# facebookarchive/Surround360

Measured on AMD Instinct MI355X. Metric: stereo-equirect frames/sec at 8K, 17-cam rig, higher is better.
Workload: dtype f32

## Files before the change

### surround360_amd/csrc/flow_kernels.hip

```cpp
#include "flow_kernels.hpp"

#include <stdexcept>

#include "devmath.hpp"

namespace s360 {

typedef float f4a8 __attribute__((ext_vector_type(4), aligned(8)));

__global__ __launch_bounds__(256) void k_resize_cubic_u8c4(const uchar4* __restrict__ src, int sw, int sh,
                                                           size_t sbs, uchar4* __restrict__ dst, int dw, int dh,
                                                           size_t dbs, double scx, double scy,
                                                           const uchar4* const* __restrict__ src_tab) {
  __shared__ int s_sx[32], s_sy[8];
  __shared__ short s_ax[32][4], s_ay[8][4];
  const int tid = threadIdx.y * blockDim.x + threadIdx.x;
  if (tid < 40) {
    const bool col = tid < 32;
    const int k = col ? tid : tid - 32;
    const int d = col ? min((int)(blockIdx.x * 32 + k), dw - 1) : min((int)(blockIdx.y * 8 + k), dh - 1);
    int s0;
    float f, cb[4];
    resize_coord(d, col ? scx : scy, &s0, &f);
    cubic_coeffs(f, cb);
    if (col) s_sx[k] = s0; else s_sy[k] = s0;
#pragma unroll
    for (int q = 0; q < 4; ++q) (col ? s_ax[k] : s_ay[k])[q] = (short)sat_s16(cv_round(cb[q] * 2048.f));
  }
  __syncthreads();
  const int dx = blockIdx.x * blockDim.x + threadIdx.x;
  const int dy = blockIdx.y * blockDim.y + threadIdx.y;
  if (dx >= dw || dy >= dh) return;
  src = src_tab ? src_tab[blockIdx.z] : src + sbs * blockIdx.z;
  dst += dbs * blockIdx.z;
  const int sx = s_sx[threadIdx.x], sy = s_sy[threadIdx.y];
  int ax[4], ay[4];
#pragma unroll
  for (int k = 0; k < 4; ++k) { ax[k] = s_ax[threadIdx.x][k]; ay[k] = s_ay[threadIdx.y][k]; }
  typedef short s16x2 __attribute__((ext_vector_type(2)));
  const s16x2 w01 = __builtin_bit_cast(s16x2, (unsigned)(ax[0] & 0xffff) | ((unsigned)ax[1] << 16));
  const s16x2 w23 = __builtin_bit_cast(s16x2, (unsigned)(ax[2] & 0xffff) | ((unsigned)ax[3] << 16));
  const int c0 = clip_idx(sx - 1, sw), c1 = clip_idx(sx, sw), c2 = clip_idx(sx + 1, sw), c3 = clip_idx(sx + 2, sw);
  int hx[4], hy[4], hz[4], hw[4];
#pragma unroll
  for (int r = 0; r < 4; ++r) {
    const unsigned* S = reinterpret_cast<const unsigned*>(src + (size_t)clip_idx(sy - 1 + r, sh) * sw);
    const unsigned p0 = S[c0], p1 = S[c1], p2 = S[c2], p3 = S[c3];
    int h[4];
#pragma unroll
    for (int ch = 0; ch < 4; ++ch) {
      const unsigned sel = 0x0c040c00u + ch * 0x00010001u;
      const s16x2 lo = __builtin_bit_cast(s16x2, __builtin_amdgcn_perm(p1, p0, sel));
      const s16x2 hi = __builtin_bit_cast(s16x2, __builtin_amdgcn_perm(p3, p2, sel));
      h[ch] = __builtin_amdgcn_sdot2(lo, w01, 0, false);
      h[ch] = __builtin_amdgcn_sdot2(hi, w23, h[ch], false);
    }
    hx[r] = h[0]; hy[r] = h[1]; hz[r] = h[2]; hw[r] = h[3];
  }
  uchar4 o;
  if (dx < (dw & ~1)) {
    const float scale = 1.f / (2048 * 2048);
    const float b0 = (float)ay[0] * scale, b1 = (float)ay[1] * scale, b2 = (float)ay[2] * scale, b3 = (float)ay[3] * scale;
    auto vf = [&](const int* hh) {
      float s = (float)hh[0] * b0;
      s = s + (float)hh[1] * b1;
      s = s + (float)hh[2] * b2;
      s = s + (float)hh[3] * b3;
      return (unsigned char)sat_u8(cv_round(s));
    };
    o.x = vf(hx); o.y = vf(hy); o.z = vf(hz); o.w = vf(hw);
  } else {
    auto vi = [&](const int* hh) {
      const int v = __mul24(hh[0], ay[0]) + __mul24(hh[1], ay[1]) + __mul24(hh[2], ay[2]) + __mul24(hh[3], ay[3]);
      return (unsigned char)sat_u8((v + (1 << 21)) >> 22);
    };
    o.x = vi(hx); o.y = vi(hy); o.z = vi(hz); o.w = vi(hw);
  }
  dst[(size_t)dy * dw + dx] = o;
}

__global__ __launch_bounds__(256) void k_gray_alpha(const uchar4* __restrict__ src, size_t n, size_t sbs,
                                                    float* __restrict__ gray, float* __restrict__ alpha,
                                                    size_t pbs) {
  const size_t i = (size_t)blockIdx.x * blockDim.x + threadIdx.x;
  if (i >= n) return;
  const uchar4 p = src[sbs * blockIdx.z + i];
  const float inv255 = (float)(1.0 / 255.0);
  const int g = (p.x * 1868 + p.y * 9617 + p.z * 4899 + (1 << 13)) >> 14;
  gray[pbs * blockIdx.z + i] = (float)g * inv255;
  alpha[pbs * blockIdx.z + i] = (float)p.w * inv255;
}

__global__ __launch_bounds__(256) void k_motion(const uchar4* __restrict__ cur, const uchar4* __restrict__ prev,
                                                size_t n, size_t sbs, float* __restrict__ motion, size_t pbs) {
  const size_t i = (size_t)blockIdx.x * blockDim.x + threadIdx.x;
  if (i >= n) return;
  const uchar4 a = cur[sbs * blockIdx.z + i], b = prev[sbs * blockIdx.z + i];
  const double s = fabs((double)((int)a.x - (int)b.x)) + fabs((double)((int)a.y - (int)b.y)) +
                   fabs((double)((int)a.z - (int)b.z));
  motion[pbs * blockIdx.z + i] = (float)(s / (double)(255.0f * 3.0f));
}

struct UpSrc {
  int sw, sh;
  size_t sbs;
  double scx, scy;
  float post_scale;
};
template <int R, int CN, int EPI, int SRC, int SB_TW = 64, int SB_TH = 16, int NT = 256>
__global__ __launch_bounds__(NT) void k_sepblur(const float* __restrict__ src, float* __restrict__ dst, int w, int h,
                                                 size_t bs , BlurTaps taps,
                                                 const float* __restrict__ A, FlowIdx idx,
                                                 const float2* __restrict__ Gp, void* __restrict__ recv,
                                                 float* const* __restrict__ dst_tab, UpSrc up,
                                                 unsigned* __restrict__ rowflags) {
  constexpr int IW = SB_TW + 2 * R, IH = SB_TH + 2 * R;
  constexpr int IWP = IW | 1;
  __shared__ __attribute__((aligned(8))) float s_in[IH][IWP][CN];
  __shared__ __attribute__((aligned(8))) float s_mid[IH][SB_TW + 1][CN];
  const int tid = threadIdx.y * blockDim.x + threadIdx.x;
  const TileId tile = xcd_tile();
  const int tx0 = tile.x * SB_TW, ty0 = tile.y * SB_TH;
  const int vecEnd = ((w * CN) / 8) * 8;
  constexpr int kColTasks = SB_TW * (SB_TH / 4);
  static_assert(EPI == 0 || kColTasks <= NT, "one column task per thread when the epilogue is prefetched");
  float pa0[4] = {0.f, 0.f, 0.f, 0.f}, pa1[4] = {0.f, 0.f, 0.f, 0.f}, pm[4] = {0.f, 0.f, 0.f, 0.f};
  float2 pg[4];
  if (EPI != 0 && tid < kColTasks) {
    const int lx = tid % SB_TW, ly0 = (tid / SB_TW) * 4, gx = tx0 + lx;
    const size_t b0 = bs * idx.i0[tile.z], b1 = bs * idx.i1[tile.z];
#pragma unroll
    for (int o = 0; o < 4; ++o) {
      const int gy = ty0 + ly0 + o;
      pg[o] = make_float2(0.f, 0.f);
      if (gx < w && gy < h) {
        const size_t off = (size_t)gy * w + gx;
        pa0[o] = A[b0 + off];
        pa1[o] = A[b1 + off];
        if (EPI == 3) pg[o] = Gp[b0 + off];
        if (EPI == 4) {
          pg[o] = Gp[bs * tile.z + off];
          pm[o] = static_cast<const float*>(recv)[b1 + off];
        }
      }
    }
  }
  src += (SRC == 2 ? up.sbs * CN : bs * (SRC == 1 ? 1 : CN)) * tile.z;
  constexpr int LW = (IW + 7) & ~7;
  constexpr bool kColumnWalk = (NT % LW) == 0;
  const int lxc = tid % LW, lyc = tid / LW;
  const int gxc = reflect101(tx0 - R + (lxc < IW ? lxc : 0), w);
  constexpr int kLdStep = kColumnWalk ? NT / LW : NT, kLdEnd = kColumnWalk ? IH : IH * IW;
  constexpr int kLdIters = (kLdEnd + kLdStep - 1) / kLdStep;
  float ld[kLdIters][CN];
#pragma unroll
  for (int it = 0; it < kLdIters; ++it) {
    const int i = min((kColumnWalk ? lyc : tid) + it * kLdStep, kLdEnd - 1);
    const int ly = kColumnWalk ? i : i / IW, lx = kColumnWalk ? min(lxc, IW - 1) : i - ly * IW;
    const int gy = reflect101(ty0 - R + ly, h), gx = kColumnWalk ? gxc : reflect101(tx0 - R + lx, w);
    if (SRC == 2) {
      int sx, sy;
      float fx, fy;
      resize_coord(gx, up.scx, &sx, &fx);
      if (sx < 0) { fx = 0; sx = 0; }
      if (sx >= up.sw - 1) { fx = 0; sx = up.sw - 1; }
      resize_coord(gy, up.scy, &sy, &fy);
      const float* S0 = src + (size_t)clip_idx(sy, up.sh) * up.sw * CN;
      const float* S1 = src + (size_t)clip_idx(sy + 1, up.sh) * up.sw * CN;
      const float b0 = 1.f - fy, b1 = fy;
#pragma unroll
      for (int k = 0; k < CN; ++k) {
        float h0, h1;
        if (sx >= up.sw - 1) {
          h0 = S0[sx * CN + k] * 1.0f;
          h1 = S1[sx * CN + k] * 1.0f;
        } else {
          const float a0 = 1.f - fx, a1 = fx;
          h0 = S0[sx * CN + k] * a0 + S0[(sx + 1) * CN + k] * a1;
          h1 = S1[sx * CN + k] * a0 + S1[(sx + 1) * CN + k] * a1;
        }
        float v = h0 * b0 + h1 * b1;
        v *= up.post_scale;
        ld[it][k] = v;
      }
    } else if (SRC == 1) {
      const float* r0 = src + (size_t)gy * w;
      ld[it][0] = r0[min(gx + 1, w - 1)] - r0[max(gx - 1, 0)];
      ld[it][CN - 1] = src[(size_t)min(gy + 1, h - 1) * w + gx] - src[(size_t)max(gy - 1, 0) * w + gx];
    } else if (CN == 2) {
      const float2 v = *reinterpret_cast<const float2*>(src + ((size_t)gy * w + gx) * CN);
      ld[it][0] = v.x;
      ld[it][CN - 1] = v.y;
    } else {
      ld[it][0] = src[(size_t)gy * w + gx];
    }
  }
#pragma unroll
  for (int it = 0; it < kLdIters; ++it) {
    const int i = (kColumnWalk ? lyc : tid) + it * kLdStep;
    if (i >= kLdEnd || (kColumnWalk && lxc >= IW)) continue;
    const int ly = kColumnWalk ? i : i / IW, lx = kColumnWalk ? lxc : i - ly * IW;
    if (CN == 2) *reinterpret_cast<float2*>(&s_in[ly][lx][0]) = make_float2(ld[it][0], ld[it][CN - 1]);
    else s_in[ly][lx][0] = ld[it][0];
  }
  __syncthreads();
  for (int t = tid; t < IH * (SB_TW / 4); t += NT) {
    const int ly = t % IH, lx0 = (t / IH) * 4;
    float v[CN][4 + 2 * R];
#pragma unroll
    for (int j = 0; j < 4 + 2 * R; ++j) {
      if (CN == 2) {
        const float2 p = *reinterpret_cast<const float2*>(&s_in[ly][lx0 + j][0]);
        v[0][j] = p.x;
        v[CN - 1][j] = p.y;
      } else {
        v[0][j] = s_in[ly][lx0 + j][0];
      }
    }
#pragma unroll
    for (int o = 0; o < 4; ++o) {
      float acc[CN];
#pragma unroll
      for (int k = 0; k < CN; ++k) {
        if (R <= 2) {
          acc[k] = taps.k[0] * v[k][o + R];
#pragma unroll
          for (int j = 1; j <= R; ++j) acc[k] += taps.k[j] * (v[k][o + R + j] + v[k][o + R - j]);
        } else {
          acc[k] = ((tx0 + lx0 + o) * CN + k < vecEnd) ? 0.0f : -0.0f;
#pragma unroll
          for (int j = 0; j <= 2 * R; ++j) acc[k] += taps.k[j < R ? R - j : j - R] * v[k][o + j];
        }
      }
      if (CN == 2) *reinterpret_cast<float2*>(&s_mid[ly][lx0 + o][0]) = make_float2(acc[0], acc[CN - 1]);
      else s_mid[ly][lx0 + o][0] = acc[0];
    }
  }
  __syncthreads();
  dst = dst_tab ? dst_tab[tile.z] : dst + bs * CN * tile.z;
  for (int t = tid; t < SB_TW * (SB_TH / 4); t += NT) {
    const int lx = t % SB_TW, ly0 = (t / SB_TW) * 4;
    const int gx = tx0 + lx;
    float outv[4][CN];
    {
      float v[CN][4 + 2 * R];
#pragma unroll
      for (int j = 0; j < 4 + 2 * R; ++j) {
        if (CN == 2) {
          const float2 p = *reinterpret_cast<const float2*>(&s_mid[ly0 + j][lx][0]);
          v[0][j] = p.x;
          v[CN - 1][j] = p.y;
        } else {
          v[0][j] = s_mid[ly0 + j][lx][0];
        }
      }
      if (CN == 2) {
        typedef float f32x2 __attribute__((ext_vector_type(2)));
        f32x2 p[4 + 2 * R];
#pragma unroll
        for (int j = 0; j < 4 + 2 * R; ++j) p[j] = f32x2{v[0][j], v[CN - 1][j]};
#pragma unroll
        for (int o = 0; o < 4; ++o) {
          f32x2 acc = taps.k[0] * p[o + R] + 0.0f;
#pragma unroll
          for (int j = 1; j <= R; ++j) acc += taps.k[j] * (p[o + R + j] + p[o + R - j]);
          outv[o][0] = acc.x;
          outv[o][CN - 1] = acc.y;
        }
      } else {
#pragma unroll
        for (int k = 0; k < CN; ++k)
#pragma unroll
          for (int o = 0; o < 4; ++o) {
            float acc = taps.k[0] * v[k][o + R] + 0.0f;
#pragma unroll
            for (int j = 1; j <= R; ++j) acc += taps.k[j] * (v[k][o + R + j] + v[k][o + R - j]);
            outv[o][k] = acc;
          }
      }
    }
    if (gx >= w) continue;
#pragma unroll
    for (int o = 0; o < 4; ++o) {
      const int gy = ty0 + ly0 + o;
      if (gy >= h) continue;
      const size_t off = (size_t)gy * w + gx;
      if (EPI == 1 || EPI == 4) {
        const float cc = 1.0f - pa0[o] * pa1[o];
#pragma unroll
        for (int k = 0; k < CN; ++k) outv[o][k] = cc * outv[o][k] + (1.0f - cc) * s_in[ly0 + o + R][lx + R][k];
      }
      if (EPI == 4) {
        const float wgt = 1.0f - pm[o];
        const float px = pg[o].x * up.post_scale, py = pg[o].y * up.post_scale;
        outv[o][0] = outv[o][0] * (1.0f - wgt) + px * wgt;
        outv[o][CN - 1] = outv[o][CN - 1] * (1.0f - wgt) + py * wgt;
      }
      if (EPI == 2 || EPI == 3) {
        const bool upd = pa0[o] > 0.9f && pa1[o] > 0.9f;
        if (EPI == 2)
          static_cast<float2*>(recv)[bs * tile.z + off] = make_float2(upd ? outv[o][0] : __int_as_float(0x7fc00000), outv[o][CN - 1]);
        else
          static_cast<float4*>(recv)[bs * tile.z + off] = make_float4(upd ? pg[o].x : __int_as_float(0x7fc00000), pg[o].y, outv[o][0], outv[o][CN - 1]);
        if (rowflags && upd) rowflags[(size_t)tile.z * h + gy] = 0u;
      } else {
#pragma unroll
        for (int k = 0; k < CN; ++k) dst[off * CN + k] = outv[o][k];
      }
    }
  }
}

template <int CN, int PPT>
__global__ __launch_bounds__(256) void k_resize_linear_f32(const float* __restrict__ src, int sw, int sh, size_t sbs,
                                                           float* __restrict__ dst, int dw, int dh, size_t dbs,
                                                           double scx, double scy, float post_scale, int do_scale) {
  const int dx = blockIdx.x * blockDim.x + threadIdx.x;
  const int dy = blockIdx.y * blockDim.y + threadIdx.y;
  if (dx >= dw || dy >= dh) return;
  int sx, sy;
  float fx, fy;
  resize_coord(dx, scx, &sx, &fx);
  if (sx < 0) { fx = 0; sx = 0; }
  if (sx >= sw - 1) { fx = 0; sx = sw - 1; }
  resize_coord(dy, scy, &sy, &fy);
  const size_t r0 = (size_t)clip_idx(sy, sh) * sw * CN, r1 = (size_t)clip_idx(sy + 1, sh) * sw * CN;
  const float b0 = 1.f - fy, b1 = fy;
  const bool edge = sx >= sw - 1;
  const int sx1 = edge ? sx : sx + 1;
  const float a0 = 1.f - fx, a1 = fx;
  float t[PPT][CN][4];
#pragma unroll
  for (int pl = 0; pl < PPT; ++pl) {
    const size_t z = (size_t)blockIdx.z * PPT + pl;
    const float* S0 = src + sbs * CN * z + r0;
    const float* S1 = src + sbs * CN * z + r1;
#pragma unroll
    for (int k = 0; k < CN; ++k) {
      t[pl][k][0] = S0[sx * CN + k];
      t[pl][k][1] = S0[sx1 * CN + k];
      t[pl][k][2] = S1[sx * CN + k];
      t[pl][k][3] = S1[sx1 * CN + k];
    }
  }
#pragma unroll
  for (int pl = 0; pl < PPT; ++pl) {
    const size_t z = (size_t)blockIdx.z * PPT + pl;
    float* D = dst + dbs * CN * z;
#pragma unroll
    for (int k = 0; k < CN; ++k) {
      float h0, h1;
      if (edge) {
        h0 = t[pl][k][0] * 1.0f;
        h1 = t[pl][k][2] * 1.0f;
      } else {
        h0 = t[pl][k][0] * a0 + t[pl][k][1] * a1;
        h1 = t[pl][k][2] * a0 + t[pl][k][3] * a1;
      }
      float v = h0 * b0 + h1 * b1;
      if (do_scale) v *= post_scale;
      D[((size_t)dy * dw + dx) * CN + k] = v;
    }
  }
}

constexpr int RL_TW = 64, RL_TH = 16, RL_BW = 76, RL_BH = 20;
template <int PPT>
__global__ __launch_bounds__(256) void k_resize_linear_f32c1_tiled(const float* __restrict__ src, int sw, int sh, size_t sbs,
                                                                   float* __restrict__ dst, int dw, int dh, size_t dbs,
                                                                   double scx, double scy, float post_scale, int do_scale) {
  __shared__ __attribute__((aligned(16))) float s_box[PPT][RL_BH][RL_BW];
  __shared__ int s_sx[RL_TW], s_r0[RL_TH], s_r1[RL_TH];
  __shared__ float s_fx[RL_TW], s_fy[RL_TH];
  const TileId tile = xcd_tile();
  const int tid = threadIdx.x, tx0 = tile.x * RL_TW, ty0 = tile.y * RL_TH;
  if (tid < RL_TW) {
    int sx;
    float fx;
    resize_coord(min(tx0 + tid, dw - 1), scx, &sx, &fx);
    if (sx < 0) { fx = 0; sx = 0; }
    if (sx >= sw - 1) { fx = 0; sx = sw - 1; }
    s_sx[tid] = sx;
    s_fx[tid] = fx;
  } else if (tid < RL_TW + RL_TH) {
    int sy;
    float fy;
    resize_coord(min(ty0 + tid - RL_TW, dh - 1), scy, &sy, &fy);
    s_r0[tid - RL_TW] = clip_idx(sy, sh);
    s_r1[tid - RL_TW] = clip_idx(sy + 1, sh);
    s_fy[tid - RL_TW] = fy;
  }
  __syncthreads();
  const int bx0 = s_sx[0], by0 = s_r0[0];
  const int bw4 = (min(s_sx[RL_TW - 1] + 1, sw - 1) - bx0 + 4) >> 2, bh = s_r1[RL_TH - 1] - by0 + 1;
  const int npieces = bh * bw4;
  constexpr int kIters = (RL_BH * (RL_BW / 4) + 255) / 256;
  float4 ld[kIters][PPT];
#pragma unroll
  for (int it = 0; it < kIters; ++it) {
    const int i = min(tid + it * 256, npieces - 1);
    const int row = i / bw4, gx = bx0 + 4 * (i - row * bw4);
    const size_t off = (size_t)(by0 + row) * sw;
#pragma unroll
    for (int pl = 0; pl < PPT; ++pl) {
      const float* S = src + sbs * ((size_t)tile.z * PPT + pl) + off;
      if (gx + 3 < sw) {
        typedef float f4a4 __attribute__((ext_vector_type(4), aligned(4)));
        const f4a4 q = *reinterpret_cast<const f4a4*>(S + gx);
        ld[it][pl] = make_float4(q.x, q.y, q.z, q.w);
      } else {
        ld[it][pl] = make_float4(S[min(gx, sw - 1)], S[min(gx + 1, sw - 1)], S[min(gx + 2, sw - 1)], S[sw - 1]);
      }
    }
  }
#pragma unroll
  for (int it = 0; it < kIters; ++it) {
    const int i = tid + it * 256;
    if (i >= npieces) continue;
    const int row = i / bw4, c4 = i - row * bw4;
#pragma unroll
    for (int pl = 0; pl < PPT; ++pl) *reinterpret_cast<float4*>(&s_box[pl][row][4 * c4]) = ld[it][pl];
  }
  __syncthreads();
  const int cx = tid & (RL_TW - 1), dx = tx0 + cx;
  if (dx >= dw) return;
  const int sxa = s_sx[cx], sxr = sxa - bx0;
  const bool edge = sxa >= sw - 1;
  const int sx1 = edge ? sxr : sxr + 1;
  const float fx = s_fx[cx], a0 = 1.f - fx, a1 = fx;
#pragma unroll
  for (int j = 0; j < RL_TH / 4; ++j) {
    const int ry = (tid >> 6) + 4 * j, dy = ty0 + ry;
    if (dy >= dh) continue;
    const int r0 = s_r0[ry] - by0, r1 = s_r1[ry] - by0;
    const float fy = s_fy[ry], b0 = 1.f - fy, b1 = fy;
#pragma unroll
    for (int pl = 0; pl < PPT; ++pl) {
      const float t0 = s_box[pl][r0][sxr], t1 = s_box[pl][r0][sx1], t2 = s_box[pl][r1][sxr], t3 = s_box[pl][r1][sx1];
      float h0, h1;
      if (edge) {
        h0 = t0 * 1.0f;
        h1 = t2 * 1.0f;
      } else {
        h0 = t0 * a0 + t1 * a1;
        h1 = t2 * a0 + t3 * a1;
      }
      float v = h0 * b0 + h1 * b1;
      if (do_scale) v *= post_scale;
      dst[dbs * ((size_t)tile.z * PPT + pl) + (size_t)dy * dw + dx] = v;
    }
  }
}

__global__ __launch_bounds__(256) void k_resize_cubic_f32c2(const float2* __restrict__ src, int sw, int sh,
                                                            size_t sbs, float2* __restrict__ dst, int dw, int dh,
                                                            size_t dbs, double scx, double scy, float post_scale,
                                                            const float2* const* __restrict__ src_tab) {
  const int dx = blockIdx.x * blockDim.x + threadIdx.x;
  const int dy = blockIdx.y * blockDim.y + threadIdx.y;
  if (dx >= dw || dy >= dh) return;
  src = src_tab ? src_tab[blockIdx.z] : src + sbs * blockIdx.z;
  dst += dbs * blockIdx.z;
  int sx, sy;
  float fx, fy, ax[4], ay[4];
  resize_coord(dx, scx, &sx, &fx);
  cubic_coeffs(fx, ax);
  resize_coord(dy, scy, &sy, &fy);
  cubic_coeffs(fy, ay);
  const int x0 = clip_idx(sx - 1, sw), x1 = clip_idx(sx, sw), x2 = clip_idx(sx + 1, sw), x3 = clip_idx(sx + 2, sw);
  float hx[4], hy[4];
#pragma unroll
  for (int r = 0; r < 4; ++r) {
    const float2* S = src + (size_t)clip_idx(sy - 1 + r, sh) * sw;
    const float2 p0 = S[x0], p1 = S[x1], p2 = S[x2], p3 = S[x3];
    hx[r] = p0.x * ax[0] + p1.x * ax[1] + p2.x * ax[2] + p3.x * ax[3];
    hy[r] = p0.y * ax[0] + p1.y * ax[1] + p2.y * ax[2] + p3.y * ax[3];
  }
  float2 o;
  o.x = hx[0] * ay[0] + hx[1] * ay[1] + hx[2] * ay[2] + hx[3] * ay[3];
  o.y = hy[0] * ay[0] + hy[1] * ay[1] + hy[2] * ay[2] + hy[3] * ay[3];
  o.x *= post_scale;
  o.y *= post_scale;
  dst[(size_t)dy * dw + dx] = o;
}

constexpr int UC_TW = 64, UC_TH = 16, UC_SW = 72, UC_SH = 24;
__global__ __launch_bounds__(256) void k_resize_cubic_f32c2_tiled(const float2* __restrict__ src, int sw, int sh,
                                                                  size_t sbs, float2* __restrict__ dst, int dw, int dh,
                                                                  size_t dbs, double scx, double scy, float post_scale) {
  __shared__ float2 s_src[UC_SH][UC_SW];
  __shared__ float2 s_h[UC_SH][UC_TW];
  __shared__ float s_ax[UC_TW][4], s_ay[UC_TH][4];
  __shared__ int s_sx[UC_TW], s_sy[UC_TH];
  const int tid = threadIdx.x;
  const TileId tile = xcd_tile();
  const int dx0 = tile.x * UC_TW, dy0 = tile.y * UC_TH;
  src += sbs * tile.z;
  dst += dbs * tile.z;
  if (tid < UC_TW) {
    float f;
    resize_coord(min(dx0 + tid, dw - 1), scx, &s_sx[tid], &f);
    cubic_coeffs(f, s_ax[tid]);
  } else if (tid < UC_TW + UC_TH) {
    float f;
    resize_coord(min(dy0 + tid - UC_TW, dh - 1), scy, &s_sy[tid - UC_TW], &f);
    cubic_coeffs(f, s_ay[tid - UC_TW]);
  }
  __syncthreads();
  const int X0 = clip_idx(s_sx[0] - 1, sw), X1 = clip_idx(s_sx[UC_TW - 1] + 2, sw);
  const int Y0 = clip_idx(s_sy[0] - 1, sh), Y1 = clip_idx(s_sy[UC_TH - 1] + 2, sh);
  const int W = X1 - X0 + 1, H = Y1 - Y0 + 1;
  const int c = tid & (UC_TW - 1), q = tid >> 6;
  {
    constexpr int kIt = (UC_SH + 3) / 4;
    float2 v[kIt];
#pragma unroll
    for (int it = 0; it < kIt; ++it) {
      const int ly = q + 4 * it;
      v[it] = (ly < H && c < W) ? src[(size_t)(Y0 + ly) * sw + X0 + c] : make_float2(0.f, 0.f);
    }
#pragma unroll
    for (int it = 0; it < kIt; ++it) {
      const int ly = q + 4 * it;
      if (ly < H && c < W) s_src[ly][c] = v[it];
    }
  }
  if (W > UC_TW) {
    const int lx = UC_TW + (tid & 7);
    for (int ly = tid >> 3; ly < H; ly += 32)
      if (lx < W) s_src[ly][lx] = src[(size_t)(Y0 + ly) * sw + X0 + lx];
  }
  __syncthreads();
  {
    const int sx = s_sx[c];
    const int o0 = clip_idx(sx - 1, sw) - X0, o1 = clip_idx(sx, sw) - X0, o2 = clip_idx(sx + 1, sw) - X0,
              o3 = clip_idx(sx + 2, sw) - X0;
    const float a0 = s_ax[c][0], a1 = s_ax[c][1], a2 = s_ax[c][2], a3 = s_ax[c][3];
    for (int ly = q; ly < H; ly += 4) {
      const float2 p0 = s_src[ly][o0], p1 = s_src[ly][o1], p2 = s_src[ly][o2], p3 = s_src[ly][o3];
      float2 hv;
      hv.x = p0.x * a0 + p1.x * a1 + p2.x * a2 + p3.x * a3;
      hv.y = p0.y * a0 + p1.y * a1 + p2.y * a2 + p3.y * a3;
      s_h[ly][c] = hv;
    }
  }
  __syncthreads();
  const int r0 = q * 4;
  const int dx = dx0 + c;
  if (dx >= dw) return;
#pragma unroll
  for (int j = 0; j < 4; ++j) {
    const int r = r0 + j, dy = dy0 + r;
    if (dy >= dh) break;
    const int sy = s_sy[r];
    const float2 h0 = s_h[clip_idx(sy - 1, sh) - Y0][c], h1 = s_h[clip_idx(sy, sh) - Y0][c],
                 h2 = s_h[clip_idx(sy + 1, sh) - Y0][c], h3 = s_h[clip_idx(sy + 2, sh) - Y0][c];
    const float b0 = s_ay[r][0], b1 = s_ay[r][1], b2 = s_ay[r][2], b3 = s_ay[r][3];
    float2 o;
    o.x = h0.x * b0 + h1.x * b1 + h2.x * b2 + h3.x * b3;
    o.y = h0.y * b0 + h1.y * b1 + h2.y * b2 + h3.y * b3;
    o.x *= post_scale;
    o.y *= post_scale;
    dst[(size_t)dy * dw + dx] = o;
  }
}




__global__ void k_search_init(const float* __restrict__ I, const float* __restrict__ A, int w, int h, size_t pbs,
                              FlowIdx idx, float2* __restrict__ flow, int hint, int dist, float* __restrict__ I1eq) {
  const int b = blockIdx.x;
  const float* __restrict__ I0 = I + pbs * idx.i0[b];
  const float* __restrict__ I1 = I + pbs * idx.i1[b];
  const float* __restrict__ A0 = A + pbs * idx.i0[b];
  const float* __restrict__ A1 = A + pbs * idx.i1[b];
  flow += pbs * b;
  I1eq += pbs * b;
  __shared__ float s_ratio;
  if (threadIdx.x == 0) {
    float sumL = 0, sumR = 0;
    for (int i = 0; i < w * h; ++i) {
      const float a = A0[i] * A1[i];
      sumL += a * I0[i];
      sumR += a * I1[i];
    }
    s_ratio = sumL / sumR;
  }
  __syncthreads();
  const float ratio = s_ratio;
  for (int i = threadIdx.x; i < w * h; i += blockDim.x) I1eq[i] = I1[i] * ratio;
  __syncthreads();
  const int kRatio = 8;
  const int ortho = (dist + kRatio / 2) / kRatio;
  const int thickness = 2 * ortho + 1;
  int bx, by, bw, bh;
  if (hint == 1) { bx = 0; by = -ortho; bw = dist + 1; bh = thickness; }
  else if (hint == 2) { bx = -ortho; by = 0; bw = thickness; bh = dist + 1; }
  else if (hint == 3) { bx = -dist; by = -ortho; bw = dist + 1; bh = thickness; }
  else { bx = -ortho; by = -dist; bw = thickness; bh = dist + 1; }
  auto patchErr = [&](int i0x, int i0y, int i1x, int i1y) -> float {
    float sad = 0, alpha = 0;
    for (int dy = -2; dy <= 2; ++dy) {
      const int d0y = i0y + dy;
      if (0 <= d0y && d0y < h) {
        const int d1y = min(max(i1y + dy, 0), h - 1);
        for (int dx = -2; dx <= 2; ++dx) {
          const int d0x = i0x + dx;
          if (0 <= d0x && d0x < w) {
            const int d1x = min(max(i1x + dx, 0), w - 1);
            const float difference = I0[d0y * w + d0x] - I1eq[d1y * w + d1x];
            sad += fabsf(difference);
            alpha += A0[d0y * w + d0x] * A1[d1y * w + d1x];
          }
        }
      }
    }
    sad /= alpha;
    const float ddx = (float)(i1x - i0x), ddy = (float)(i1y - i0y);
    const float length = (float)sqrt((double)ddx * ddx + (double)ddy * ddy);
    sad *= 1 + length / dist;
    return sad;
  };
  for (int i = threadIdx.x; i < w * h; i += blockDim.x) {
    const int i0y = i / w, i0x = i - i0y * w;
    if (A0[i] > 0.9f) {
      float errorBest = 0.8f * patchErr(i0x, i0y, i0x, i0y);
      int bxb = i0x, byb = i0y;
      for (int dy = by; dy < by + bh; ++dy)
        for (int dx = bx; dx < bx + bw; ++dx) {
          const int i1x = i0x + dx, i1y = i0y + dy;
          if (0 <= i1x && i1x < w && 0 <= i1y && i1y < h) {
            const float e = patchErr(i0x, i0y, i1x, i1y);
            if (errorBest > e) { errorBest = e; bxb = i1x; byb = i1y; }
          }
        }
      flow[i] = make_float2((float)(bxb - i0x), (float)(byb - i0y));
    }
  }
}

static inline dim3 grid2d(int w, int h, int B, dim3 blk) { return dim3((w + blk.x - 1) / blk.x, (h + blk.y - 1) / blk.y, B); }

void launch_resize_cubic_u8c4(hipStream_t st, const uchar4* src, int sw, int sh, size_t sbs, uchar4* dst, int dw,
                              int dh, size_t dbs, int B, const uchar4* const* src_tab) {
  const double scx = 1.0 / ((double)dw / (double)sw), scy = 1.0 / ((double)dh / (double)sh);
  dim3 blk(32, 8);
  hipLaunchKernelGGL(k_resize_cubic_u8c4, grid2d(dw, dh, B, blk), blk, 0, st, src, sw, sh, sbs, dst, dw, dh, dbs, scx,
                     scy, src_tab);
}
void launch_gray_alpha(hipStream_t st, const uchar4* src, size_t n, size_t sbs, float* gray, float* alpha, size_t pbs,
                       int B) {
  hipLaunchKernelGGL(k_gray_alpha, dim3((unsigned)((n + 255) / 256), 1, B), dim3(256), 0, st, src, n, sbs, gray, alpha,
                     pbs);
}
void launch_motion(hipStream_t st, const uchar4* cur, const uchar4* prev, size_t n, size_t sbs, float* motion,
                   size_t pbs, int B) {
  hipLaunchKernelGGL(k_motion, dim3((unsigned)((n + 255) / 256), 1, B), dim3(256), 0, st, cur, prev, n, sbs, motion,
                     pbs);
}
template <int R, int CN, int EPI, int SRC>
static void launch_sepblur_t(hipStream_t st, const float* src, float* dst, int w, int h, size_t bs, int B,
                             const BlurTaps& t, const float* A, const FlowIdx& idx, const float2* Gp, void* rec,
                             float* const* dst_tab = nullptr, const UpSrc& up = UpSrc{}, unsigned* rowflags = nullptr) {
  dim3 blk(64, 4);
  if constexpr (R == 7) {
    dim3 grd((w + 31) / 32, (h + 31) / 32, B);
    hipLaunchKernelGGL((k_sepblur<R, CN, EPI, SRC, 32, 32, 384>), grd, dim3(64, 6), 0, st, src, dst, w, h, bs, t, A, idx, Gp, rec, dst_tab, up, rowflags);
  } else {
    dim3 grd((w + 63) / 64, (h + 15) / 16, B);
    hipLaunchKernelGGL((k_sepblur<R, CN, EPI, SRC>), grd, blk, 0, st, src, dst, w, h, bs, t, A, idx, Gp, rec, dst_tab, up, rowflags);
  }
}
void launch_sepblur(hipStream_t st, const float* src, float* dst, int w, int h, int cn, size_t bs, int B,
                    const BlurTaps& t, float* const* dst_tab) {
  static const FlowIdx none = {nullptr, nullptr};
  if (t.r == 1 && cn == 1) launch_sepblur_t<1, 1, 0, 0>(st, src, dst, w, h, bs, B, t, nullptr, none, nullptr, nullptr);
  else if (t.r == 1 && cn == 2) launch_sepblur_t<1, 2, 0, 0>(st, src, dst, w, h, bs, B, t, nullptr, none, nullptr, nullptr, dst_tab);
  else if (t.r == 2 && cn == 1) launch_sepblur_t<2, 1, 0, 0>(st, src, dst, w, h, bs, B, t, nullptr, none, nullptr, nullptr);
  else if (t.r == 7 && cn == 2) launch_sepblur_t<7, 2, 0, 0>(st, src, dst, w, h, bs, B, t, nullptr, none, nullptr, nullptr);
  else throw std::runtime_error("launch_sepblur: unsupported radius/channels");
}
void launch_diffusion(hipStream_t st, const float2* flow, float2* dst, int w, int h, size_t bs, int B,
                      const BlurTaps& t, const float* A, const FlowIdx& idx) {
  launch_sepblur_t<7, 2, 1, 0>(st, (const float*)flow, (float*)dst, w, h, bs, B, t, A, idx, nullptr, nullptr);
}
void launch_diffusion_adjust(hipStream_t st, const float2* flow, float2* dst, int w, int h, size_t bs, int B, const BlurTaps& t,
                             const float* A, const FlowIdx& idx, const float2* prev, const float* motion, float prev_scale) {
  UpSrc up{};
  up.post_scale = prev_scale;
  launch_sepblur_t<7, 2, 4, 0>(st, (const float*)flow, (float*)dst, w, h, bs, B, t, A, idx, prev, const_cast<float*>(motion), nullptr, up);
}
void launch_upscale_blur(hipStream_t st, const float2* src, int sw, int sh, size_t sbs, float2* dst, int dw, int dh,
                         size_t dbs, int B, float post_scale, const BlurTaps& t, float* const* dst_tab) {
  static const FlowIdx none = {nullptr, nullptr};
  if (t.r != 1) throw std::runtime_error("launch_upscale_blur: 3x3 kernel expected");
  UpSrc up;
  up.sw = sw; up.sh = sh; up.sbs = sbs;
  up.scx = 1.0 / ((double)dw / (double)sw);
  up.scy = 1.0 / ((double)dh / (double)sh);
  up.post_scale = post_scale;
  launch_sepblur_t<1, 2, 0, 2>(st, (const float*)src, (float*)dst, dw, dh, dbs, B, t, nullptr, none, nullptr, nullptr, dst_tab, up);
}
void launch_gradients(hipStream_t st, const float* I, float2* G, int w, int h, size_t bs, int B, const BlurTaps& t) {
  static const FlowIdx none = {nullptr, nullptr};
  if (t.r != 1) throw std::runtime_error("launch_gradients: 3x3 kernel expected");
  launch_sepblur_t<1, 2, 0, 1>(st, I, (float*)G, w, h, bs, B, t, nullptr, none, nullptr, nullptr);
}
void launch_blur_to_records(hipStream_t st, const float2* flow, void* rec, int w, int h, size_t bs, int B,
                            const BlurTaps& t, const float2* G, const float* A, const FlowIdx& idx, unsigned* rowflags) {
  if (t.r != 7) throw std::runtime_error("launch_blur_to_records: 15x15 kernel expected");
  if (G) launch_sepblur_t<7, 2, 3, 0>(st, (const float*)flow, nullptr, w, h, bs, B, t, A, idx, G, rec, nullptr, UpSrc{}, rowflags);
  else launch_sepblur_t<7, 2, 2, 0>(st, (const float*)flow, nullptr, w, h, bs, B, t, A, idx, nullptr, rec, nullptr, UpSrc{}, rowflags);
}
void launch_resize_linear_f32(hipStream_t st, const float* src, int sw, int sh, size_t sbs, float* dst, int dw, int dh,
                              size_t dbs, int cn, int B, float post_scale, int do_scale) {
  const double scx = 1.0 / ((double)dw / (double)sw), scy = 1.0 / ((double)dh / (double)sh);
  const int ppt = (B % 4 == 0) ? 4 : (B % 2 == 0) ? 2 : 1;
  const int tw = std::min(dw, RL_TW), th = std::min(dh, RL_TH);
  const bool fits = std::min(sw, (int)std::floor((tw - 1) * scx) + 3) + 3 <= RL_BW &&
                    std::min(sh, (int)std::floor((th - 1) * scy) + 3) <= RL_BH;
  if (cn == 1 && fits) {
    const dim3 grid((dw + RL_TW - 1) / RL_TW, (dh + RL_TH - 1) / RL_TH, B / ppt);
#define S360_RLT(P)                                                                                                   \
  hipLaunchKernelGGL((k_resize_linear_f32c1_tiled<P>), grid, dim3(256), 0, st, src, sw, sh, sbs, dst, dw, dh, dbs, scx, \
                     scy, post_scale, do_scale)
    if (ppt == 4) S360_RLT(4); else if (ppt == 2) S360_RLT(2); else S360_RLT(1);
#undef S360_RLT
    return;
  }
  dim3 blk(32, 8);
#define S360_RL(C, P)                                                                                                   \
  hipLaunchKernelGGL((k_resize_linear_f32<C, P>), grid2d(dw, dh, B / P, blk), blk, 0, st, src, sw, sh, sbs, dst, dw, dh, \
                     dbs, scx, scy, post_scale, do_scale)
  if (cn == 1) { if (ppt == 4) S360_RL(1, 4); else if (ppt == 2) S360_RL(1, 2); else S360_RL(1, 1); }
  else { if (ppt == 4) S360_RL(2, 4); else if (ppt == 2) S360_RL(2, 2); else S360_RL(2, 1); }
#undef S360_RL
}
void launch_resize_cubic_f32c2(hipStream_t st, const float2* src, int sw, int sh, size_t sbs, float2* dst, int dw,
                               int dh, size_t dbs, int B, float post_scale, const float2* const* src_tab) {
  const double scx = 1.0 / ((double)dw / (double)sw), scy = 1.0 / ((double)dh / (double)sh);
  if (!src_tab && scx <= 1.0 && scy <= 1.0) {
    hipLaunchKernelGGL(k_resize_cubic_f32c2_tiled, dim3((dw + UC_TW - 1) / UC_TW, (dh + UC_TH - 1) / UC_TH, B), dim3(256),
                       0, st, src, sw, sh, sbs, dst, dw, dh, dbs, scx, scy, post_scale);
    return;
  }
  dim3 blk(32, 8);
  hipLaunchKernelGGL(k_resize_cubic_f32c2, grid2d(dw, dh, B, blk), blk, 0, st, src, sw, sh, sbs, dst, dw, dh, dbs, scx,
                     scy, post_scale, src_tab);
}
void launch_search_init(hipStream_t st, const float* I, const float* A, int w, int h, size_t pbs, int B,
                        const FlowIdx& idx, float2* flow, int hint, int dist, float* I1eq) {
  hipLaunchKernelGGL(k_search_init, dim3(B), dim3(256), 0, st, I, A, w, h, pbs, idx, flow, hint, dist, I1eq);
}

}
```

### surround360_amd/csrc/flow_kernels.hpp

```cpp
#pragma once
#include <hip/hip_runtime.h>
#include <stddef.h>

#include <vector>

namespace s360 {

struct BlurTaps {
  int r;
  float k[8];
};
constexpr int kMaxFlows = 2048;
struct FlowIdx {
  const int* i0;
  const int* i1;
};
struct PixFlowConsts {
  float pyrScaleFactor, smoothnessCoef, verticalRegularizationCoef, horizontalRegularizationCoef;
  float gradientStepSize, downscaleFactor;
  int maxPercentage;
};

void launch_resize_cubic_u8c4(hipStream_t st, const uchar4* src, int sw, int sh, size_t sbs, uchar4* dst, int dw,
                              int dh, size_t dbs, int B, const uchar4* const* src_tab = nullptr);
void launch_gray_alpha(hipStream_t st, const uchar4* src, size_t n, size_t sbs, float* gray, float* alpha, size_t pbs,
                       int B);
void launch_motion(hipStream_t st, const uchar4* cur, const uchar4* prev, size_t n, size_t sbs, float* motion,
                   size_t pbs, int B);
void launch_sepblur(hipStream_t st, const float* src, float* dst, int w, int h, int cn, size_t bs, int B,
                    const BlurTaps& t, float* const* dst_tab = nullptr);
void launch_diffusion(hipStream_t st, const float2* flow, float2* dst, int w, int h, size_t bs, int B,
                      const BlurTaps& t, const float* A, const FlowIdx& idx);
void launch_diffusion_adjust(hipStream_t st, const float2* flow, float2* dst, int w, int h, size_t bs, int B, const BlurTaps& t,
                             const float* A, const FlowIdx& idx, const float2* prev, const float* motion, float prev_scale);
void launch_upscale_blur(hipStream_t st, const float2* src, int sw, int sh, size_t sbs, float2* dst, int dw, int dh,
                         size_t dbs, int B, float post_scale, const BlurTaps& t, float* const* dst_tab = nullptr);
void launch_gradients(hipStream_t st, const float* I, float2* G, int w, int h, size_t bs, int B, const BlurTaps& t);
void launch_blur_to_records(hipStream_t st, const float2* flow, void* rec, int w, int h, size_t bs, int B,
                            const BlurTaps& t, const float2* G, const float* A, const FlowIdx& idx,
                            unsigned* rowflags = nullptr);
void launch_resize_linear_f32(hipStream_t st, const float* src, int sw, int sh, size_t sbs, float* dst, int dw, int dh,
                              size_t dbs, int cn, int B, float post_scale, int do_scale);
void launch_resize_cubic_f32c2(hipStream_t st, const float2* src, int sw, int sh, size_t sbs, float2* dst, int dw,
                               int dh, size_t dbs, int B, float post_scale, const float2* const* src_tab = nullptr);
void launch_median5_c2(hipStream_t st, const float2* src, float2* dst, int w, int h, size_t bs, int B);
int sweep_lock_waves();
int sweep_lock_num_wgs(int h, int nw);
size_t sweep_lock_handoff_bytes(int w, int h, int B, int nw);
void launch_sweep_lock(hipStream_t st, const float4* rec, const float2* G, float2* flow, void* handoff,
                       unsigned* errflag, int w, int h, size_t bs, int B, const FlowIdx& idx, int dir,
                       const PixFlowConsts& pc, bool fast);
bool sweep_verify_divisors(hipStream_t st, const std::vector<float>& divisors);
size_t sweep_quad_handoff_bytes(int w, int h, int B);
void launch_sweep_quad(hipStream_t st, const float2* rec, const float2* G, float2* flow, void* handoff,
                       unsigned* errflag, int w, int h, size_t bs, int B, const FlowIdx& idx, int dir,
                       const PixFlowConsts& pc, bool fast, const unsigned* rowflags = nullptr);
void launch_search_init(hipStream_t st, const float* I, const float* A, int w, int h, size_t pbs, int B,
                        const FlowIdx& idx, float2* flow, int hint, int dist, float* I1eq);

}
```

Measured before the change: 48.88.

## Skip blur tiles with no valid alpha and add horizontal-only cubic resize kernel

Adds a fast path in the epilogue blur variants: each block votes on whether any pixel has both alphas above threshold. If none do, it writes sentinel records (NaN marker) and returns without blurring. It also adds a specialised horizontal-only cubic resize kernel for the case where the source and destination heights match. That kernel stages a row box in LDS and uses packed sdot2 integer filtering. Both paths are on by default behind an environment toggle, and they depend on downstream kernels handling the sentinel records correctly.

Result: faster. 49.89 (median of 6 runs) (+2.1%).

```diff
diff --git a/surround360_amd/csrc/flow_kernels.hip b/surround360_amd/csrc/flow_kernels.hip
--- a/surround360_amd/csrc/flow_kernels.hip
+++ b/surround360_amd/csrc/flow_kernels.hip
@@ -1,5 +1,7 @@
 #include "flow_kernels.hpp"
 
+#include <cmath>
+#include <cstdlib>
 #include <stdexcept>
 
 #include "devmath.hpp"
@@ -79,6 +81,92 @@
   dst[(size_t)dy * dw + dx] = o;
 }
 
+constexpr int HR_TW = 256, HR_TH = 16, HR_BW = 320;
+typedef unsigned u32x4a4 __attribute__((ext_vector_type(4), aligned(4)));
+typedef unsigned u32x4 __attribute__((ext_vector_type(4)));
+__global__ __launch_bounds__(256) void k_resize_cubic_u8c4_h(const uchar4* __restrict__ src, int sw, int h, size_t sbs,
+                                                             uchar4* __restrict__ dst, int dw, size_t dbs, double scx) {
+  __shared__ __attribute__((aligned(16))) unsigned s_box[HR_TH][HR_BW];
+  const int tid = threadIdx.x, cx = tid & 63, q = tid >> 6;
+  const int tx0 = blockIdx.x * HR_TW, ty0 = blockIdx.y * HR_TH;
+  const unsigned* S = reinterpret_cast<const unsigned*>(src + sbs * blockIdx.z);
+  unsigned* D = reinterpret_cast<unsigned*>(dst + dbs * blockIdx.z);
+  int s0, s1;
+  float f;
+  resize_coord(min(tx0, dw - 1), scx, &s0, &f);
+  resize_coord(min(tx0 + HR_TW - 1, dw - 1), scx, &s1, &f);
+  const int bx0 = clip_idx(s0 - 1, sw) & ~3, bx1 = clip_idx(s1 + 2, sw);
+  const int np4 = (bx1 - bx0 + 4) >> 2, npieces = HR_TH * np4;
+  constexpr int kIters = (HR_TH * (HR_BW / 4) + 255) / 256;
+  u32x4a4 ld[kIters];
+#pragma unroll
+  for (int it = 0; it < kIters; ++it) {
+    const int i = min(tid + it * 256, npieces - 1);
+    const int row = i / np4, gx = bx0 + 4 * (i - row * np4);
+    const unsigned* Sr = S + (size_t)min(ty0 + row, h - 1) * sw;
+    if (gx + 3 < sw) ld[it] = *reinterpret_cast<const u32x4a4*>(Sr + gx);
+    else ld[it] = u32x4a4{Sr[min(gx, sw - 1)], Sr[min(gx + 1, sw - 1)], Sr[min(gx + 2, sw - 1)], Sr[sw - 1]};
+  }
+#pragma unroll
+  for (int it = 0; it < kIters; ++it) {
+    const int i = tid + it * 256;
+    if (i >= npieces) continue;
+    const int row = i / np4, c4 = i - row * np4;
+    *reinterpret_cast<u32x4*>(&s_box[row][4 * c4]) = u32x4{ld[it].x, ld[it].y, ld[it].z, ld[it].w};
+  }
+  typedef short s16x2 __attribute__((ext_vector_type(2)));
+  const int dx0 = tx0 + 4 * cx;
+  int c[4][4];
+  s16x2 w01[4], w23[4];
+#pragma unroll
+  for (int j = 0; j < 4; ++j) {
+    int sx;
+    float cb[4];
+    resize_coord(min(dx0 + j, dw - 1), scx, &sx, &f);
+    cubic_coeffs(f, cb);
+    int a[4];
+#pragma unroll
+    for (int k = 0; k < 4; ++k) {
+      a[k] = sat_s16(cv_round(cb[k] * 2048.f));
+      c[j][k] = clip_idx(sx - 1 + k, sw) - bx0;
+    }
+    w01[j] = __builtin_bit_cast(s16x2, (unsigned)(a[0] & 0xffff) | ((unsigned)a[1] << 16));
+    w23[j] = __builtin_bit_cast(s16x2, (unsigned)(a[2] & 0xffff) | ((unsigned)a[3] << 16));
+  }
+  __syncthreads();
+  if (dx0 >= dw) return;
+#pragma unroll
+  for (int r = 0; r < HR_TH / 4; ++r) {
+    const int row = q * (HR_TH / 4) + r, dy = ty0 + row;
+    if (dy >= h) break;
+    unsigned o[4];
+#pragma unroll
+    for (int j = 0; j < 4; ++j) {
+      const unsigned p0 = s_box[row][c[j][0]], p1 = s_box[row][c[j][1]], p2 = s_box[row][c[j][2]], p3 = s_box[row][c[j][3]];
+      const bool sse = dx0 + j < (dw & ~1);
+      o[j] = 0;
+#pragma unroll
+      for (int ch = 0; ch < 4; ++ch) {
+        const unsigned sel = 0x0c040c00u + ch * 0x00010001u;
+        const s16x2 lo = __builtin_bit_cast(s16x2, __builtin_amdgcn_perm(p1, p0, sel));
+        const s16x2 hi = __builtin_bit_cast(s16x2, __builtin_amdgcn_perm(p3, p2, sel));
+        int h1 = __builtin_amdgcn_sdot2(lo, w01[j], 0, false);
+        h1 = __builtin_amdgcn_sdot2(hi, w23[j], h1, false);
+        const int v = sse ? (int)__builtin_rintf((float)h1 * (1.f / 2048)) : (h1 * 2048 + (1 << 21)) >> 22;
+        o[j] |= (unsigned)sat_u8(v) << (8 * ch);
+      }
+    }
+    unsigned* Dr = D + (size_t)dy * dw + dx0;
+    if (dx0 + 3 < dw) {
+      *reinterpret_cast<u32x4a4*>(Dr) = u32x4a4{o[0], o[1], o[2], o[3]};
+    } else {
+#pragma unroll
+      for (int j = 0; j < 4; ++j)
+        if (dx0 + j < dw) Dr[j] = o[j];
+    }
+  }
+}
+
 __global__ __launch_bounds__(256) void k_gray_alpha(const uchar4* __restrict__ src, size_t n, size_t sbs,
                                                     float* __restrict__ gray, float* __restrict__ alpha,
                                                     size_t pbs) {
@@ -101,6 +189,10 @@
   motion[pbs * blockIdx.z + i] = (float)(s / (double)(255.0f * 3.0f));
 }
 
+#ifdef S360_WAVE_EMULATION
+unsigned long long g_known_stats[2];
+#define S360_KSTAT(i) __atomic_fetch_add(&g_known_stats[i], 1ull, __ATOMIC_RELAXED)
+#endif
 struct UpSrc {
   int sw, sh;
   size_t sbs;
@@ -113,7 +205,7 @@
                                                  const float* __restrict__ A, FlowIdx idx,
                                                  const float2* __restrict__ Gp, void* __restrict__ recv,
                                                  float* const* __restrict__ dst_tab, UpSrc up,
-                                                 unsigned* __restrict__ rowflags) {
+                                                 unsigned* __restrict__ rowflags, int known_result) {
   constexpr int IW = SB_TW + 2 * R, IH = SB_TH + 2 * R;
   constexpr int IWP = IW | 1;
   __shared__ __attribute__((aligned(8))) float s_in[IH][IWP][CN];
@@ -203,7 +295,37 @@
     if (CN == 2) *reinterpret_cast<float2*>(&s_in[ly][lx][0]) = make_float2(ld[it][0], ld[it][CN - 1]);
     else s_in[ly][lx][0] = ld[it][0];
   }
-  __syncthreads();
+  if constexpr (EPI == 2 || EPI == 3) {
+    __shared__ int s_vote[NT / 64];
+    bool none = true;
+#pragma unroll
+    for (int o = 0; o < 4; ++o) none &= !(pa0[o] > 0.9f && pa1[o] > 0.9f);
+    s_vote[tid >> 6] = __ballot(!none) == 0ull;
+    __syncthreads();
+    int v = known_result != 0;
+#pragma unroll
+    for (int q = 0; q < NT / 64; ++q) v &= s_vote[q];
+    const bool known = __builtin_amdgcn_readfirstlane(v) != 0;
+#ifdef S360_WAVE_EMULATION
+    if (tid == 0) S360_KSTAT(known ? 0 : 1);
+#endif
+    if (known) {
+      if (tid < kColTasks) {
+        const int lx = tid % SB_TW, ly0 = (tid / SB_TW) * 4, gx = tx0 + lx;
+#pragma unroll
+        for (int o = 0; o < 4; ++o) {
+          const int gy = ty0 + ly0 + o;
+          if (gx >= w || gy >= h) continue;
+          const size_t off = (size_t)gy * w + gx;
+          if (EPI == 2) static_cast<float2*>(recv)[bs * tile.z + off] = make_float2(__int_as_float(0x7fc00000), 0.0f);
+          else static_cast<float4*>(recv)[bs * tile.z + off] = make_float4(__int_as_float(0x7fc00000), pg[o].y, 0.0f, 0.0f);
+        }
+      }
+      return;
+    }
+  } else {
+    __syncthreads();
+  }
   for (int t = tid; t < IH * (SB_TW / 4); t += NT) {
     const int ly = t % IH, lx0 = (t / IH) * 4;
     float v[CN][4 + 2 * R];
@@ -640,11 +762,24 @@
   }
 }
 
+bool known_result_enabled() {
+  static const bool on = [] {
+    const char* e = std::getenv("S360_KNOWN_RESULT");
+    return !(e && e[0] == '0' && e[1] == 0);
+  }();
+  return on;
+}
+
 static inline dim3 grid2d(int w, int h, int B, dim3 blk) { return dim3((w + blk.x - 1) / blk.x, (h + blk.y - 1) / blk.y, B); }
 
 void launch_resize_cubic_u8c4(hipStream_t st, const uchar4* src, int sw, int sh, size_t sbs, uchar4* dst, int dw,
                               int dh, size_t dbs, int B, const uchar4* const* src_tab) {
   const double scx = 1.0 / ((double)dw / (double)sw), scy = 1.0 / ((double)dh / (double)sh);
+  if (sh == dh && !src_tab && known_result_enabled() && (int)std::ceil((HR_TW - 1) * scx) + 12 <= HR_BW) {
+    hipLaunchKernelGGL(k_resize_cubic_u8c4_h, dim3((dw + HR_TW - 1) / HR_TW, (dh + HR_TH - 1) / HR_TH, B), dim3(256), 0, st,
+                       src, sw, sh, sbs, dst, dw, dbs, scx);
+    return;
+  }
   dim3 blk(32, 8);
   hipLaunchKernelGGL(k_resize_cubic_u8c4, grid2d(dw, dh, B, blk), blk, 0, st, src, sw, sh, sbs, dst, dw, dh, dbs, scx,
                      scy, src_tab);
@@ -666,10 +801,10 @@
   dim3 blk(64, 4);
   if constexpr (R == 7) {
     dim3 grd((w + 31) / 32, (h + 31) / 32, B);
-    hipLaunchKernelGGL((k_sepblur<R, CN, EPI, SRC, 32, 32, 384>), grd, dim3(64, 6), 0, st, src, dst, w, h, bs, t, A, idx, Gp, rec, dst_tab, up, rowflags);
+    hipLaunchKernelGGL((k_sepblur<R, CN, EPI, SRC, 32, 32, 384>), grd, dim3(64, 6), 0, st, src, dst, w, h, bs, t, A, idx, Gp, rec, dst_tab, up, rowflags, known_result_enabled() ? 1 : 0);
   } else {
     dim3 grd((w + 63) / 64, (h + 15) / 16, B);
-    hipLaunchKernelGGL((k_sepblur<R, CN, EPI, SRC>), grd, blk, 0, st, src, dst, w, h, bs, t, A, idx, Gp, rec, dst_tab, up, rowflags);
+    hipLaunchKernelGGL((k_sepblur<R, CN, EPI, SRC>), grd, blk, 0, st, src, dst, w, h, bs, t, A, idx, Gp, rec, dst_tab, up, rowflags, known_result_enabled() ? 1 : 0);
   }
 }
 void launch_sepblur(hipStream_t st, const float* src, float* dst, int w, int h, int cn, size_t bs, int B,
diff --git a/surround360_amd/csrc/flow_kernels.hpp b/surround360_amd/csrc/flow_kernels.hpp
--- a/surround360_amd/csrc/flow_kernels.hpp
+++ b/surround360_amd/csrc/flow_kernels.hpp
@@ -20,6 +20,11 @@
   float gradientStepSize, downscaleFactor;
   int maxPercentage;
 };
+
+bool known_result_enabled();
+#ifdef S360_WAVE_EMULATION
+extern unsigned long long g_known_stats[2];
+#endif
 
 void launch_resize_cubic_u8c4(hipStream_t st, const uchar4* src, int sw, int sh, size_t sbs, uchar4* dst, int dw,
                               int dh, size_t dbs, int B, const uchar4* const* src_tab = nullptr);
```
